# team-charls/charls

Hardware: AMD Instinct MI355X
Metric: MPixels/s encode+decode, 4096x4096 8-bit gray, bit-exact vs CharLS (higher is better)
Workload: dtype u8

## Files before the change

### charls_amd/csrc/device/tile_pipeline.hip

```cpp
#pragma once
#include <hip/hip_runtime.h>

#include <algorithm>
#include <cstdlib>

#include "pipeline_common.hip"

namespace jls {
namespace tile {

using pipe::kChains;
using pipe::kInterruptChain;
using pipe::kNoEvent;
using pipe::kStatusInvalid;
using pipe::kZeroContextChain;


constexpr uint32_t kMaxTileSamples = 8192;
constexpr uint32_t kTileLines = 16;
constexpr uint32_t kSegments = 16;
constexpr uint32_t kThreads = 512;
constexpr uint32_t kWaves = kThreads / 64;
constexpr uint32_t kPackThreads = 512;
constexpr uint16_t kNoLocalSlot = 0xFFFF;
// ... 1551 lines not shown
    return w.run_jobs[jobs].type1 < w.run_jobs[jobs].type0;
}

template <typename S, int FMT>
__global__ void __launch_bounds__(64) compact_rare_runs(const Work* __restrict__ works)
{
    const Work w = works[blockIdx.y];
    const uint32_t n = w.chain_total[0];
    const uint32_t jobs = (n + w.run_job_events - 1) / w.run_job_events;
    if (jobs == 0)
        return;
    const uint32_t* runs = reinterpret_cast<const uint32_t*>(rec_slots<S>(w) + w.chain_base[0]);
    const Slot<S>* int_rec = rec_slots<S>(w) + w.chain_base[kInterruptChain];
    int32_t* rare = reinterpret_cast<int32_t*>(w.code);
    const int rare_type = rarer_is_type1(w, jobs) ? 1 : 0;
    const int lane = threadIdx.x;
    for (uint32_t job = blockIdx.x; job < jobs; job += gridDim.x)
    {
        const uint32_t from = job * w.run_job_events;
        const uint32_t to = from + w.run_job_events < n ? from + w.run_job_events : n;
        const RunJob mine = w.run_jobs[job];
        uint32_t at = rare_type ? mine.type1 : mine.type0, own_at = mine.own_slot;
        for (uint32_t e0 = from; e0 < to; e0 += 64)
        {
            const uint32_t e = e0 + (uint32_t)lane;
            const uint32_t v = e < to ? runs[e] : 0u;
            bool is_rare, own;
            if (FMT == 1)
            {
                const bool interrupted = e < to && !RunRecord2::is_end_of_line(v);
                is_rare = interrupted && RunRecord2::which(v) == rare_type;
                own = interrupted && !RunRecord2::is_zero_run(v);
            }
            else
            {
                const bool interrupted = e < to && !RunRecord<S>::is_end_of_line(v);
                is_rare = interrupted && RunRecord<S>::which(v) == rare_type;
                own = interrupted && RunRecord<S>::run(v) != 0;
            }
            const unsigned long long rare_m = __ballot(is_rare), own_m = __ballot(own);
            const unsigned long long below = (1ull << lane) - 1ull;
            if (is_rare)
            {
                int err;
                if (FMT == 1)
                    err = own ? interruption_err<S>(int_rec[own_at + (uint32_t)__popcll(own_m & below)]) : RunRecord2::err(v);
                else
                    err = RunRecord<S>::err(v);
                rare[at + (uint32_t)__popcll(rare_m & below)] = err;
            }
            at += (uint32_t)__popcll(rare_m);
            own_at += (uint32_t)__popcll(own_m);
        }
    }
}

JLS_DEV void walk_rare_context_serially(const Traits& t, const Work& w, uint32_t jobs, bool rare1)
{
    const int32_t* rare = reinterpret_cast<const int32_t*>(w.code);
    RunCtx ctx{rare1 ? 1 : 0, initial_a(t), 1, 0};
    uint32_t i = 0;
    for (uint32_t j = 0; j < jobs; ++j)
    {
        w.run_jobs[j].rare_a = ctx.a;
        w.run_jobs[j].rare_nn = ctx.nn;
        const uint32_t upto = rare1 ? w.run_jobs[j + 1].type1 : w.run_jobs[j + 1].type0;
        for (; i < upto; ++i)
        {
            const int err = rare[i];
            const int k = run_k_of_encoder(ctx);
            const int em = 2 * (err < 0 ? -err : err) - ctx.ritype - run_map(ctx, err, k);
            run_update(ctx, err, em, t.reset);
        }
    }
}

constexpr uint32_t kRareSegment = 128;
JLS_DEV void walk_rare_context(const ScanDesc& d, const Work& w)
{
    const uint32_t lane = threadIdx.x;
    const Traits t = make_traits(d);
    const uint32_t n = w.chain_total[0];
    const uint32_t jobs = (n + w.run_job_events - 1) / w.run_job_events;
    if (jobs == 0)
        return;
    const bool rare1 = rarer_is_type1(w, jobs);
    auto starts_at = [&](uint32_t j) -> uint32_t { return rare1 ? w.run_jobs[j].type1 : w.run_jobs[j].type0; };
    const uint32_t total = starts_at(jobs);
    const uint32_t per_lane = (total + 63) / 64;
    const uint32_t segment = per_lane > kRareSegment ? per_lane : kRareSegment;
    const uint32_t s = lane * segment < total ? lane * segment : total;
    const uint32_t e = s + segment < total ? s + segment : total;
    const bool active = lane == 0 || s < total;
    const bool last = e == total;
    const int32_t* rare = reinterpret_cast<const int32_t*>(w.code);
    const uint32_t warm_from = s > w.rare_warm_events ? s - w.rare_warm_events : 0u;
    RunCtx ctx{rare1 ? 1 : 0, initial_a(t), chain_n_before(warm_from, (uint32_t)t.reset), 0};
    auto one = [&](uint32_t i) {
        const int err = rare[i];
        const int k = run_k_of_encoder(ctx);
        const int em = 2 * (err < 0 ? -err : err) - ctx.ritype - run_map(ctx, err, k);
        run_update(ctx, err, em, t.reset);
    };
    int in_a = 0, in_nn = 0;
    if (active)
    {
        for (uint32_t i = warm_from; i < s; ++i)
            one(i);
        in_a = ctx.a;
        in_nn = ctx.nn;
        uint32_t lo = 0, hi = jobs;
        while (lo < hi)
        {
            const uint32_t mid = (lo + hi) / 2;
            if (starts_at(mid) < s)
                lo = mid + 1;
            else
                hi = mid;
        }
        uint32_t j = lo, next = j < jobs ? starts_at(j) : ~0u;
        for (uint32_t i = s;; ++i)
        {
            while (j < jobs && next == i && (i < e || last))
            {
                w.run_jobs[j].rare_a = ctx.a;
                w.run_jobs[j].rare_nn = ctx.nn;
                ++j;
                next = j < jobs ? starts_at(j) : ~0u;
            }
            if (i >= e)
                break;
            one(i);
        }
    }
    const int before_a = __shfl_up(ctx.a, 1), before_nn = __shfl_up(ctx.nn, 1);
    const bool differs = active && lane != 0 && (in_a != before_a || in_nn != before_nn);
    const unsigned long long guessed = __ballot(active && lane != 0);
    const bool again = __any(differs);
    if (lane == 0)
    {
        if (guessed)
            atomicAdd(&w.counters[kCountRareSegments], (uint32_t)__popcll(guessed));
        if (again)
        {
            atomicAdd(&w.counters[kCountRareSerial], 1u);
            walk_rare_context_serially(t, w, jobs, rare1);
        }
    }
}

template <typename S, int ILV, int FMT = 0>
__global__ void __launch_bounds__(64) warm_run_jobs(const ScanDesc* __restrict__ descs, const Work* __restrict__ works, uint32_t scans,
                                                    uint32_t rare_blocks)
{
    if (blockIdx.x < rare_blocks)
    {
        walk_rare_context(descs[blockIdx.x], works[blockIdx.x]);
        return;
    }
    const uint32_t tid = (blockIdx.x - rare_blocks) * 64u + threadIdx.x;
    const uint32_t job = tid / scans, frame = tid % scans;
    const ScanDesc d = descs[frame];
    const Work w = works[frame];
    const uint32_t n = w.chain_total[0];
    const uint32_t from = job * w.run_job_events;
    if (from >= n)
        return;
    const Traits t = make_traits(d);
    const uint32_t* runs = reinterpret_cast<const uint32_t*>(rec_slots<S>(w) + w.chain_base[0]);
    uint32_t* run_code = reinterpret_cast<uint32_t*>(code_slots<S>(w) + w.chain_base[0]);
    Slot<S>* int_code = code_slots<S>(w) + w.chain_base[kInterruptChain];
    const Slot<S>* int_rec = rec_slots<S>(w) + w.chain_base[kInterruptChain];
    const uint32_t warm_jobs = (w.run_warm_events + w.run_job_events - 1) / w.run_job_events;
    const uint32_t warm_job = job > warm_jobs ? job - warm_jobs : 0u;
    RunState s{0, initial_a(t), 0, initial_a(t), 0};
    if (warm_job < job)
    {
        const RunJob before = w.run_jobs[warm_job];
        walk_runs<S, ILV, false, FMT>(t, runs, run_code, int_code, warm_job * w.run_job_events, from, s, before.type0, before.type1, before.own_slot, int_rec,
                                      samples_per_pixel(d));
    }
    w.run_jobs[job].in = s;
}

template <typename S, int ILV, int FMT = 0>
__global__ void __launch_bounds__(64) walk_run_jobs(const ScanDesc* __restrict__ descs, const Work* __restrict__ works, uint32_t scans)
{
    const uint32_t tid = blockIdx.x * 64u + threadIdx.x;
    const uint32_t job = tid / scans, frame = tid % scans;
    const ScanDesc d = descs[frame];
    const Work w = works[frame];
    const uint32_t n = w.chain_total[0];
    const uint32_t from = job * w.run_job_events;
    if (from >= n)
        return;
    const Traits t = make_traits(d);
    const uint32_t to = from + w.run_job_events < n ? from + w.run_job_events : n;
    const uint32_t* runs = reinterpret_cast<const uint32_t*>(rec_slots<S>(w) + w.chain_base[0]);
    uint32_t* run_code = reinterpret_cast<uint32_t*>(code_slots<S>(w) + w.chain_base[0]);
    Slot<S>* int_code = code_slots<S>(w) + w.chain_base[kInterruptChain];
    const Slot<S>* int_rec = rec_slots<S>(w) + w.chain_base[kInterruptChain];
    const uint32_t nc = samples_per_pixel(d);
    const uint32_t jobs = (n + w.run_job_events - 1) / w.run_job_events;
    RunJob mine = w.run_jobs[job];
    RunState s = mine.in;
    if (ILV != 2)
    {
        if (rarer_is_type1(w, jobs))
        {
            s.a1 = mine.rare_a;
            s.nn1 = mine.rare_nn;
        }
        else
        {
            s.a0 = mine.rare_a;
            s.nn0 = mine.rare_nn;
        }
    }
    mine.in = s;
    walk_runs<S, ILV, true, FMT>(t, runs, run_code, int_code, from, to, s, mine.type0, mine.type1, mine.own_slot, int_rec, nc);
    mine.out = s;
    w.run_jobs[job] = mine;
}

template <typename S, int ILV, int FMT = 0>
__global__ void __launch_bounds__(64) settle_runs(const ScanDesc* __restrict__ descs, const Work* __restrict__ works, uint32_t scans)
{
    const uint32_t frame = blockIdx.x;
    if (frame >= scans)
        return;
    const ScanDesc d = descs[frame];
    const Work w = works[frame];
    const Traits t = make_traits(d);
    const uint32_t n = w.chain_total[0];
    const uint32_t jobs = (n + w.run_job_events - 1) / w.run_job_events;
    {
        bool differs = false;
        for (uint32_t j = 1 + threadIdx.x; j < jobs; j += 64)
            differs = differs || !same_state(w.run_jobs[j].in, w.run_jobs[j - 1].out);
        if (!__any(differs))
        {
            if (threadIdx.x == 0)
                atomicAdd(&w.counters[kCountRunJobs], jobs);
            return;
        }
        if (threadIdx.x != 0)
            return;
    }
    const uint32_t* runs = reinterpret_cast<const uint32_t*>(rec_slots<S>(w) + w.chain_base[0]);
    uint32_t* run_code = reinterpret_cast<uint32_t*>(code_slots<S>(w) + w.chain_base[0]);
    Slot<S>* int_code = code_slots<S>(w) + w.chain_base[kInterruptChain];
    const Slot<S>* int_rec = rec_slots<S>(w) + w.chain_base[kInterruptChain];
    const uint32_t nc = samples_per_pixel(d);
    RunState prev = w.run_jobs[0].out;
    uint32_t rewalked = 0;
    for (uint32_t j = 1; j < jobs; ++j)
    {
        const RunJob cur = w.run_jobs[j];
        RunState out = cur.out;
        if (!same_state(cur.in, prev))
        {
            ++rewalked;
            out = prev;
            const uint32_t from = j * w.run_job_events;
            const uint32_t to = from + w.run_job_events < n ? from + w.run_job_events : n;
            walk_runs<S, ILV, true, FMT>(t, runs, run_code, int_code, from, to, out, cur.type0, cur.type1, cur.own_slot, int_rec, nc);
        }
        prev = out;
    }
    atomicAdd(&w.counters[kCountRunJobs], jobs);
    if (rewalked)
        atomicAdd(&w.counters[kCountRunJobsRewalked], rewalked);
}

#define JLS_HOST_DEV __host__ __device__ inline
JLS_HOST_DEV uint32_t pack_bits_offset(uint32_t tile_capacity, uint32_t sample_bytes)
{
    const uint32_t codes = (uint32_t)stage_bytes(tile_capacity, sample_bytes);
    const uint32_t head = ((codes + 3u) & ~3u) + kPackThreads * 4 + 16 * 4 + kPieceWords * 4;
    return ((head + 15u) & ~15u) + kPieceRows * 16;
}

JLS_HOST_DEV uint32_t pack_bits_words(uint32_t tile_capacity, int32_t bits_per_sample)
{
    const uint32_t limit = 2u * (uint32_t)(bits_per_sample + (bits_per_sample > 8 ? bits_per_sample : 8));
    return tile_capacity * limit / 32 + 2;
}

JLS_DEV void expand_code(uint32_t word, uint64_t& bits, int& len)
{
    if (word & kRunTag)
    {
        const int ones = (int)((word >> 25) & 63u), tail_len = (int)((word >> 20) & 31u);
        bits = ((((uint64_t)1 << ones) - 1ull) << tail_len) | (uint64_t)(word & 0xFFFFFu);
        len = ones + tail_len;
    }
    else
    {
        bits = word & 0xFFFFFFu;
        len = (int)(word >> 24);
    }
}

JLS_DEV uint32_t shifted_word(const uint32_t* bits, uint32_t i, uint32_t head, uint32_t carry)
{
    if (head == 0)
        return bits[i];
    return (i == 0 ? carry : bits[i - 1] << (32u - head)) | (bits[i] >> head);
}

typedef uint32_t UnalignedWords4 __attribute__((vector_size(16), aligned(2)));
template <typename S>
__global__ void __launch_bounds__(kPackThreads) pack_tiles(const ScanDesc* __restrict__ descs, const Work* __restrict__ works)
{
    JLS_DYNAMIC_LDS(smem);
    constexpr bool kNarrow = sizeof(Slot<S>) == 2;
    const ScanDesc d = descs[blockIdx.y];
    const Work w = works[blockIdx.y];
    const uint32_t tile = blockIdx.x;
    const uint32_t tiles = scan_tiles(d, w);
    if (tile >= tiles)
        return;
    const uint32_t tile_capacity = w.tile_capacity;
    const uint32_t threads = blockDim.x;
    const uint32_t per_thread = ((tile_capacity + threads - 1) / threads + 7u) & ~7u;
    const int lane = threadIdx.x & 63, wave = threadIdx.x >> 6;
    const uint32_t kPackWaves = threads / 64;
    Slot<S>* s_code = reinterpret_cast<Slot<S>*>(smem);
    const uint32_t code_bytes = (uint32_t)stage_bytes(tile_capacity, (uint32_t)sizeof(S));
    uint32_t* s_scan = reinterpret_cast<uint32_t*>(smem + ((code_bytes + 3u) & ~3u));
    uint32_t* s_tmp = s_scan + kPackThreads;
    uint32_t* s_pieces = s_tmp + 16;
    const uint32_t bits_offset = pack_bits_offset(tile_capacity, (uint32_t)sizeof(S));
    uint4* s_piecerows = reinterpret_cast<uint4*>(smem + bits_offset) - kPieceRows;
    uint32_t* s_bits = reinterpret_cast<uint32_t*>(smem + bits_offset);
    const TileSpan span = tile_span(d, w, tile);
    const uint32_t tile_samples = span.count;
    const auto inv = global_ptr(w.keyinv) + span.first;

    constexpr int kGroups = (int)(kMaxTileSamples / kPackThreads / 8);
    uint4 mine[kGroups];
    JLS_PHASE_BEGIN();
#pragma unroll
    for (int q = 0; q < kGroups; ++q)
    {
        const uint32_t at = threadIdx.x * per_thread + (uint32_t)q * 8;
        mine[q] = make_uint4(~0u, ~0u, ~0u, ~0u);
        if ((uint32_t)q * 8 < per_thread && at + 8 <= tile_samples)
        {
            const UnalignedWords4 v = *reinterpret_cast<const JLS_GLOBAL_AS UnalignedWords4*>(inv + at);
            mine[q] = make_uint4(v[0], v[1], v[2], v[3]);
        }
        else if ((uint32_t)q * 8 < per_thread && at < tile_samples)
        {
            uint32_t e[8];
#pragma unroll
            for (int j = 0; j < 8; ++j)
                e[j] = at + (uint32_t)j < tile_samples ? inv[at + j] : kNoLocalSlot;
            mine[q] = make_uint4(e[0] | (e[1] << 16), e[2] | (e[3] << 16), e[4] | (e[5] << 16), e[6] | (e[7] << 16));
        }
    }
    piece_tables_clear(s_piecerows, s_pieces);
    {
        uint32_t n[2] = {0, 0}, g[2] = {0, 0};
        for (int half = 0; half < 2; ++half)
        {
            const uint32_t c = threadIdx.x + (uint32_t)half * threads;
            if (c < (uint32_t)kChains)
            {
                g[half] = global_ptr(w.seg)[(size_t)tile * kChains + c];
                n[half] = global_ptr(w.seg)[(size_t)(tile + 1) * kChains + c] - g[half];
            }
        }
        uint32_t off[2] = {n[0], n[1]}, piece[2] = {n[0] != 0 ? 1u : 0u, n[1] != 0 ? 1u : 0u};
        block_exclusive_scan_pair(off, piece, kChains, s_tmp);
        for (int half = 0; half < 2; ++half)
        {
            const uint32_t c = threadIdx.x + (uint32_t)half * threads;
            if (c < (uint32_t)kChains)
            {
                if (n[half] != 0)
                    piece_tables_add(s_piecerows, s_pieces, piece[half], off[half], n[half], g[half]);
                if (c == 0)
                    s_pieces[kChains + kPieceRun] = n[half];
                if (c == (uint32_t)kChains - 1)
                    s_pieces[kChains + kPieceTotal] = off[half] + n[half];
            }
        }
    }
    JLS_PHASE(9);
    __syncthreads();
    JLS_PHASE(11);
    copy_pieces_in<Slot<S>, 16>(s_piecerows, s_pieces, global_ptr(code_slots<S>(w)), s_code, kPackWaves);
    JLS_PHASE(12);
    __syncthreads();
    JLS_PHASE(13);

    auto slot_of = [&](int q, int j) -> uint32_t {
        const uint32_t word = (j >> 1) == 0 ? mine[q].x : (j >> 1) == 1 ? mine[q].y : (j >> 1) == 2 ? mine[q].z : mine[q].w;
        return (j & 1) ? word >> 16 : word & 0xFFFFu;
    };
    const uint32_t run_slots_end = kNarrow ? s_pieces[kChains + kPieceRun] : 0u;
    auto word_of = [&](uint32_t slot) -> uint32_t {
        if (slot == kNoLocalSlot)
            return 0u;
        if (!kNarrow)
            return (uint32_t)s_code[slot];
        if (slot < run_slots_end)
            return (uint32_t)s_code[slot] | ((uint32_t)s_code[slot + 1] << 16);
        const uint32_t c = (uint32_t)s_code[slot];
        return ((c >> 10) << 24) | (c & 0x3FFu);
    };
    uint32_t words[kGroups * 8];
    uint32_t sum = 0;
#pragma unroll
    for (int q = 0; q < kGroups; ++q)
#pragma unroll
        for (int j = 0; j < 8; ++j)
        {
            const uint32_t word = word_of(slot_of(q, j));
            words[q * 8 + j] = word;
            sum += word & kRunTag ? ((word >> 25) & 63u) + ((word >> 20) & 31u) : word >> 24;
        }
    JLS_PHASE(14);
    {
        uint32_t incl = sum;
        for (int delta = 1; delta < 64; delta <<= 1)
        {
            const uint32_t up = __shfl_up(incl, delta);
            if (lane >= delta)
                incl += up;
        }
        if (lane == 63)
            s_tmp[wave] = incl;
        __syncthreads();
        uint32_t before = 0;
        for (uint32_t w2 = 0; w2 < kPackWaves; ++w2)
            before += (int)w2 < wave ? s_tmp[w2] : 0u;
        s_scan[threadIdx.x] = before + incl;
        __syncthreads();
    }
    JLS_PHASE(15);
    const uint32_t tile_bits = s_scan[threads - 1];
    if (threadIdx.x == 0)
        store_relaxed(&global_ptr(w.blockbase)[tile], (tile == 0 ? pipe::kBlockUpTo : pipe::kBlockOwn) | (uint64_t)tile_bits);
    const uint32_t local_words = (tile_bits + 31) / 32;
    for (uint32_t i = threadIdx.x; i < local_words + 1; i += threads)
        s_bits[i] = 0;
    __syncthreads();
    if (sum != 0)
    {
        const uint32_t bitpos = s_scan[threadIdx.x] - sum;
        uint32_t word_at = bitpos >> 5;
        const uint32_t first_word = word_at;
        uint32_t pending = bitpos & 31;
        uint64_t acc = 0;
        auto put = [&](uint32_t part, uint32_t n) {
            acc |= (uint64_t)part << ((64u - pending - n) & 63u);
            pending += n;
            if (pending >= 32)
            {
                const uint32_t o = (uint32_t)(acc >> 32);
                if (word_at == first_word)
                    atomicOr(&s_bits[word_at], o);
                else
                    s_bits[word_at] = o;
                acc <<= 32;
                pending -= 32;
                ++word_at;
            }
        };
#pragma unroll
        for (int q = 0; q < kGroups; ++q)
#pragma unroll
            for (int j = 0; j < 8; ++j)
            {
                const uint32_t word = words[q * 8 + j];
                if (word == 0)
                    continue;
                uint64_t v;
                int len;
                expand_code(word, v, len);
                if (len > 32)
                {
                    put((uint32_t)(v >> 32), (uint32_t)len - 32u);
                    len = 32;
                }
                put((uint32_t)v, (uint32_t)len);
            }
        if (pending > 0)
            atomicOr(&s_bits[word_at], (uint32_t)(acc >> 32));
    }
    JLS_PHASE(18);
    __syncthreads();
    JLS_PHASE(19);
    const bool last_tile = tile + 1 == tiles;
    constexpr uint64_t kTailValid = 1ull << 63;
    if (threadIdx.x < 64)
    {
        const uint64_t own = tile_bits;
        const uint32_t b = tile;
        uint64_t start = 0;
        uint32_t reach = b;
        while (reach > 0)
        {
            const bool in_window = (uint32_t)lane < reach;
            const uint32_t j = in_window ? reach - 1 - (uint32_t)lane : 0;
            uint64_t state = 0;
            do
            {
                state = in_window ? load_relaxed(&global_ptr(w.blockbase)[j]) : pipe::kBlockOwn;
            } while (__any((state >> 62) == 0));
            const unsigned long long knows = __ballot(in_window && (state >> 62) == 2);
            const int last = knows ? (int)__ffsll(knows) - 1 : 63;
            uint64_t part = in_window && lane <= last ? state & pipe::kBlockValue : 0;
            for (int delta = 32; delta > 0; delta >>= 1)
                part += __shfl_xor(part, delta);
            start += part;
            if (knows)
                break;
            reach = reach > 64 ? reach - 64 : 0;
        }
        if (lane == 0)
        {
            if (b != 0)
                store_relaxed(&global_ptr(w.blockbase)[b], pipe::kBlockUpTo | (start + own));
            if (b + 1 == tiles)
                *global_ptr(w.total_bits) = start + own;
            const uint32_t head = (uint32_t)(start & 31);
            const uint32_t tile_words = (head + tile_bits + 31) / 32;
            const bool shared_first = head != 0;
            const bool partial_last = ((head + tile_bits) & 31u) != 0 && !last_tile;
            const bool own_tail = tile_words >= 2 || !shared_first;
            if (own_tail)
                store_relaxed(&global_ptr(w.tile_tail)[tile], kTailValid | (partial_last ? shifted_word(s_bits, tile_words - 1, head, 0u) : 0u));
            uint32_t carry = 0;
            if (shared_first)
            {
                uint64_t before;
                do
                    before = load_relaxed(&global_ptr(w.tile_tail)[tile - 1]);
                while ((before & kTailValid) == 0);
                carry = (uint32_t)before;
            }
            if (!own_tail)
                store_relaxed(&global_ptr(w.tile_tail)[tile], kTailValid | (partial_last ? shifted_word(s_bits, 0, head, carry) : 0u));
            s_tmp[12] = (uint32_t)start;
            s_tmp[13] = (uint32_t)(start >> 32);
            s_tmp[14] = carry;
        }
    }
    JLS_PHASE(16);
    __syncthreads();
    JLS_PHASE(20);
    const uint64_t tile_start = (uint64_t)s_tmp[12] | ((uint64_t)s_tmp[13] << 32);
    const uint32_t head = (uint32_t)(tile_start & 31), carry = s_tmp[14];
    const uint32_t tile_words = (head + tile_bits + 31) / 32;
    const bool partial_last = ((head + tile_bits) & 31u) != 0 && !last_tile;
    const uint64_t first_global = tile_start >> 5;
    const uint32_t stored_words = partial_last ? tile_words - 1 : tile_words;
    for (uint32_t i = threadIdx.x; i < stored_words; i += threads)
    {
        const uint64_t at = first_global + i;
        if (at < w.raw_words)
            global_ptr(w.raw)[at] = __builtin_bswap32(shifted_word(s_bits, i, head, carry));
    }
    if (last_tile && threadIdx.x < 4)
    {
        const uint64_t at = first_global + tile_words + threadIdx.x;
        if (at < w.raw_words)
            global_ptr(w.raw)[at] = 0;
    }
    JLS_PHASE(21);
}

__global__ void __launch_bounds__(256) clear_pack_state(const Work* __restrict__ works, uint32_t bytes_per_scan)
{
    uint4* at = reinterpret_cast<uint4*>(works[blockIdx.y].blockbase);
    const uint32_t groups = bytes_per_scan / 16;
    for (uint32_t g = blockIdx.x * 256u + threadIdx.x; g < groups; g += gridDim.x * 256u)
        at[g] = make_uint4(0, 0, 0, 0);
}

inline size_t tile_common_lds_bytes(uint32_t width, uint32_t lines_per_tile, uint32_t sample_bytes, int interleave_mode, bool with_keys)
{
    auto up = [](size_t v) { return (v + 15) & ~size_t{15}; };
    const size_t chunks = (width + 63) / 64;
    return up(interleave_mode == 1 ? 0 : (size_t)(lines_per_tile + 1) * width * sample_bytes) +
           (with_keys ? up((size_t)lines_per_tile * width * 2) : 0) + up((size_t)lines_per_tile * chunks * 16);
}
inline size_t analyze_lds_bytes(uint32_t width, uint32_t lines_per_tile, uint32_t sample_bytes, int interleave_mode)
{
    return tile_common_lds_bytes(width, lines_per_tile, sample_bytes, interleave_mode, true) + ((size_t)kChains + 1) * 4 + pipe::kGradientTable;
}
inline size_t sort_lds_bytes(uint32_t width, uint32_t lines_per_tile, uint32_t sample_bytes, int interleave_mode)
{
    return tile_common_lds_bytes(width, lines_per_tile, sample_bytes, interleave_mode, false) + (size_t)kPieceRows * 16 +
           (size_t)sort_segments(lines_per_tile) * kChains * 4 + 16 * 4 + (size_t)kWaves * (kChains + 1) * 4 + (size_t)kPieceWords * 4 +
           stage_bytes((uint32_t)lines_per_tile * width, sample_bytes);
}
inline uint32_t pack_threads_for(uint32_t tile_capacity)
{
    const uint32_t per_thread = ((tile_capacity + kPackThreads - 1) / kPackThreads + 7u) & ~7u;
    if ((uint64_t)per_thread * kPackThreads * 4 <= (uint64_t)tile_capacity * 5)
        return kPackThreads;
    const uint32_t fewer = ((tile_capacity + per_thread - 1) / per_thread + 63u) / 64u * 64u;
    return fewer < 192u ? 192u : (fewer > kPackThreads ? kPackThreads : fewer);
}
inline size_t pack_lds_bytes(uint32_t tile_capacity, int32_t bits_per_sample)
{
    return (size_t)pack_bits_offset(tile_capacity, bits_per_sample > 8 ? 2u : 1u) + (size_t)pack_bits_words(tile_capacity, bits_per_sample) * 4;
}
struct TilePlan
{
    uint32_t mode, nc, step, lines, line_samples, lines_per_tile, segs_per_line, seg_pixels, tiles, tile_capacity, max_pixels;
    uint64_t samples;
};
inline TilePlan plan_tiles(const ScanDesc& d)
{
    TilePlan p{};
    const uint32_t sample_bytes = d.bits_per_sample > 8 ? 2u : 1u;
    uint32_t cap = sample_bytes == 1 ? kMaxTileSamples : kMaxTileSamples / 2;
    if (const long long knob = knobs::get(knobs::kTileSamples); knob != knobs::kUnset)
        cap = std::min<uint32_t>(cap, (uint32_t)std::max<long long>(64, std::min<long long>(knob, cap)));
    const bool force_pixel_mode = knobs::get_or(knobs::kPixelMode, 0) != 0;
    p.nc = d.interleave_mode == 2 ? (uint32_t)d.components : 1u;
    p.step = d.interleave_mode == 1 ? (uint32_t)d.components : 1u;
    p.lines = d.height * (d.interleave_mode == 1 ? (uint32_t)d.components : 1u);
    p.line_samples = d.width * p.nc;
    p.samples = (uint64_t)p.line_samples * p.lines;
    if (p.line_samples <= cap)
    {
        const uint32_t n = cap / p.line_samples;
        p.lines_per_tile = n < 1 ? 1 : (n > kTileLines ? kTileLines : n);
        p.segs_per_line = 1;
        p.seg_pixels = d.width;
        p.tile_capacity = p.lines_per_tile * p.line_samples;
        p.mode = d.interleave_mode != 0 || force_pixel_mode ? 2u : 0u;
    }
    else
    {
        p.lines_per_tile = 1;
        const uint32_t fit = std::min(cap, p.line_samples) / p.nc / 64 * 64;
        const uint32_t max_px = fit < 64 ? 64 : fit;
        p.segs_per_line = (d.width + max_px - 1) / max_px;
        p.seg_pixels = ((d.width + p.segs_per_line - 1) / p.segs_per_line + 63) / 64 * 64;
        p.tile_capacity = p.seg_pixels * p.nc;
        p.mode = 2;
    }
    p.tiles = (p.lines + p.lines_per_tile - 1) / p.lines_per_tile * p.segs_per_line;
    p.max_pixels = p.segs_per_line == 1 ? d.width : p.seg_pixels;
    return p;
}
}
}
```

Before: 18160.

## Pack tile bitstream with a per-thread merge tree of short codes

Adds a fast path in pack_tiles that merges each thread's sixteen codes into two 64-bit halves through a binary shift-or tree, then writes them as at most five 32-bit words. It applies only when every code in the wave fits in 32 bits and each half fits in 64 bits; otherwise the old sequential put loop runs, re-reading the slots. It aims to replace the serial per-code accumulator loop and its branches with branch-free shifts. The cost is a wave-wide vote, extra 64-bit register pressure, and duplicated slot reads on the fallback path.

```diff
diff --git a/charls_amd/csrc/device/tile_pipeline.hip b/charls_amd/csrc/device/tile_pipeline.hip
--- a/charls_amd/csrc/device/tile_pipeline.hip
+++ b/charls_amd/csrc/device/tile_pipeline.hip
@@ -1877,6 +1877,25 @@
     }
 }
 
+#ifndef JLS_PACK_TREE
+#define JLS_PACK_TREE 1
+#endif
+
+JLS_DEV void short_code(uint32_t word, uint32_t& bits, uint32_t& len)
+{
+    const uint32_t ones = (word >> 25) & 63u, tail_len = (word >> 20) & 31u;
+    const bool run = (word & kRunTag) != 0;
+    const uint32_t run_bits = ((uint32_t)(((uint64_t)1 << ones) - 1ull) << tail_len) | (word & 0xFFFFFu);
+    bits = run ? run_bits : word & 0xFFFFFFu;
+    len = run ? ones + tail_len : word >> 24;
+}
+
+JLS_DEV void merge_codes(uint64_t& bits, uint32_t& len, uint64_t left_bits, uint32_t left_len, uint64_t right_bits, uint32_t right_len)
+{
+    bits = (left_bits << (right_len & 63u)) | right_bits;
+    len = left_len + right_len;
+}
+
 JLS_DEV uint32_t shifted_word(const uint32_t* bits, uint32_t i, uint32_t head, uint32_t carry)
 {
     if (head == 0)
@@ -1986,6 +2005,43 @@
         const uint32_t c = (uint32_t)s_code[slot];
         return ((c >> 10) << 24) | (c & 0x3FFu);
     };
+#if JLS_PACK_TREE
+    static_assert(kGroups == 2, "the merge tree of pack_tiles takes two groups of eight samples per thread");
+    uint64_t half_bits[kGroups];
+    uint32_t half_len[kGroups];
+    uint32_t longest = 0;
+#pragma unroll
+    for (int q = 0; q < kGroups; ++q)
+    {
+        uint64_t pair_bits[4];
+        uint32_t pair_len[4];
+#pragma unroll
+        for (int p = 0; p < 4; ++p)
+        {
+            uint32_t b0, l0, b1, l1;
+            short_code(word_of(slot_of(q, 2 * p)), b0, l0);
+            short_code(word_of(slot_of(q, 2 * p + 1)), b1, l1);
+            const uint32_t longer = l0 > l1 ? l0 : l1;
+            longest = longest > longer ? longest : longer;
+            merge_codes(pair_bits[p], pair_len[p], b0, l0, b1, l1);
+        }
+        uint64_t four_bits[2];
+        uint32_t four_len[2];
+        merge_codes(four_bits[0], four_len[0], pair_bits[0], pair_len[0], pair_bits[1], pair_len[1]);
+        merge_codes(four_bits[1], four_len[1], pair_bits[2], pair_len[2], pair_bits[3], pair_len[3]);
+        merge_codes(half_bits[q], half_len[q], four_bits[0], four_len[0], four_bits[1], four_len[1]);
+    }
+    const uint32_t sum = half_len[0] + half_len[1];
+    const bool tree = __all(longest <= 32u && half_len[0] <= 64u && half_len[1] <= 64u);
+    const uint32_t behind = half_len[1] & 63u;
+    const bool behind_full = half_len[1] >= 64u;
+    const uint64_t tree_lo = (behind_full ? 0ull : half_bits[0] << behind) | half_bits[1];
+    const uint64_t tree_hi = behind_full ? half_bits[0] : (half_bits[0] >> 1) >> (63u - behind);
+#ifdef JLS_PATH_PROFILE
+    if (lane == 0)
+        s_tmp[8 + wave] = tree ? 1u : 0u;
+#endif
+#else
     uint32_t words[kGroups * 8];
     uint32_t sum = 0;
 #pragma unroll
@@ -1997,6 +2053,7 @@
             words[q * 8 + j] = word;
             sum += word & kRunTag ? ((word >> 25) & 63u) + ((word >> 20) & 31u) : word >> 24;
         }
+#endif
     JLS_PHASE(14);
     {
         uint32_t incl = sum;
@@ -2009,6 +2066,13 @@
         if (lane == 63)
             s_tmp[wave] = incl;
         __syncthreads();
+#if JLS_PACK_TREE && defined(JLS_PATH_PROFILE)
+        for (uint32_t w2 = 0; w2 < kPackWaves; ++w2)
+        {
+            JLS_PATH_ADD(20, s_tmp[8 + w2]);
+            JLS_PATH_ADD(21, 1u - s_tmp[8 + w2]);
+        }
+#endif
         uint32_t before = 0;
         for (uint32_t w2 = 0; w2 < kPackWaves; ++w2)
             before += (int)w2 < wave ? s_tmp[w2] : 0u;
@@ -2023,6 +2087,34 @@
     for (uint32_t i = threadIdx.x; i < local_words + 1; i += threads)
         s_bits[i] = 0;
     __syncthreads();
+#if JLS_PACK_TREE
+    if (tree)
+    {
+        if (sum != 0)
+        {
+            const uint32_t end = s_scan[threadIdx.x];
+            const uint32_t first_word = (end - sum) >> 5, last_word = (end - 1u) >> 5;
+            const uint32_t up = (0u - end) & 31u;
+            const uint64_t low = tree_lo << up;
+            const uint64_t mid = (tree_hi << up) | ((tree_lo >> 1) >> (63u - up));
+            const uint32_t top = (uint32_t)((tree_hi >> 1) >> (63u - up));
+            const uint32_t before_last = last_word - first_word;
+            atomicOr(&s_bits[last_word], (uint32_t)low);
+            if (before_last > 1)
+                s_bits[last_word - 1] = (uint32_t)(low >> 32);
+            if (before_last > 2)
+                s_bits[last_word - 2] = (uint32_t)mid;
+            if (before_last > 3)
+                s_bits[last_word - 3] = (uint32_t)(mid >> 32);
+            if (before_last != 0)
+                atomicOr(&s_bits[first_word], before_last == 1   ? (uint32_t)(low >> 32)
+                                              : before_last == 2 ? (uint32_t)mid
+                                              : before_last == 3 ? (uint32_t)(mid >> 32)
+                                                                 : top);
+        }
+    }
+    else
+#endif
     if (sum != 0)
     {
         const uint32_t bitpos = s_scan[threadIdx.x] - sum;
@@ -2050,7 +2142,11 @@
 #pragma unroll
             for (int j = 0; j < 8; ++j)
             {
+#if JLS_PACK_TREE
+                const uint32_t word = word_of(slot_of(q, j));
+#else
                 const uint32_t word = words[q * 8 + j];
+#endif
                 if (word == 0)
                     continue;
                 uint64_t v;
```

Result: no change. 18190, median of 3 (+0.1%).
